# ezwelty/glimpse

Hardware: AMD Instinct MI355X
Metric: particle-frames/s (higher is better)
Workload: dtype f64

## Files before the change

### glimpse_amd/_lib.py

```python
import ctypes as C
import os

import numpy as np

HERE = os.path.dirname(os.path.abspath(__file__))
LIB_PATH = os.environ.get("GLH_LIB") or os.path.join(HERE, "lib", "libglimpse_hip.so")

CAM_LEN = 24
MOTION_LEN = 18
MOTION_FULL_LEN = 24
MOTION_KINDS = {"cartesian": 0, "cylindrical": 1, "tangent_cartesian": 2, "tangent_cylindrical": 3, "external": 4}
RNG_HOST, RNG_PHILOX = 0, 1
MATH_EXACT, MATH_FAST = 0, 1
RESAMPLE = {"systematic": 0, "stratified": 1, "choice": 2, "residual": 3}
OK = 0
PT_NAN, PT_TEMPLATE_OOB, PT_SAMPLE_OUTSIDE, PT_RESAMPLE_CLAMP, PT_CONST_TILE = 1, 2, 4, 8, 16
PT_RASTER_OOB, PT_NOT_VISIBLE = 32, 64
RASTER_DEM, RASTER_DEM_SIGMA, RASTER_VIEWSHED = 0, 1, 2
OBS_OK, OBS_SKIPPED, OBS_OUT_OF_BOUNDS, OBS_TILE_TOO_LARGE, OBS_NO_TEMPLATE = 0, 1, 2, 3, 4
NO_ERROR_FRAME = 0x7F7F7F7F
COMM_ID_BYTES = 128


class GlhError(RuntimeError):
# ... 31 lines not shown
    "glh_sync": (_I, [_P]),
    "glh_get_stream": (_I, [_P, _P]),
    "glh_observer_init": (_I, [_P, _I, _I, _I, _I, _I, _D]),
    "glh_observer_set_cameras": (_I, [_P, _I, _I, _I, _P]),
    "glh_observer_set_depth": (_I, [_P, _I, _I]),
    "glh_observer_upload_frame": (_I, [_P, _I, _I, _P]),
    "glh_observer_upload_frame_async": (_I, [_P, _I, _I, _P]),
    "glh_host_register": (_I, [_P, _U64]),
    "glh_host_unregister": (_I, [_P]),
    "glh_observer_upload_frame_pinned": (_I, [_P, _I, _I, _P, _P]),
    "glh_upload_done": (_I, [_P, C.c_int64, _I, _P]),
    "glh_observer_set_frame_device": (_I, [_P, _I, _I, _P]),
    "glh_begin_sequence": (_I, [_P, _I, _I, _I, _I]),
    "glh_set_motion_cartesian": (_I, [_P, _P]),
    "glh_set_motion": (_I, [_P, _P]),
    "glh_set_raster": (_I, [_P, _I, _P, _I, _I, _P, _P, _I, _I, _D, _D, _D, _D]),
    "glh_set_point_offset": (_I, [_P, _I]),
    "glh_set_observer_mask": (_I, [_P, _P]),
    "glh_set_active": (_I, [_P, _P]),
    "glh_set_particles": (_I, [_P, _P]),
    "glh_get_particles": (_I, [_P, _P]),
    "glh_set_weights": (_I, [_P, _P]),
    "glh_get_weights": (_I, [_P, _P]),
    "glh_set_extra_log_likelihoods": (_I, [_P, _P]),
    "glh_get_point_status": (_I, [_P, _P]),
    "glh_get_point_error_frame": (_I, [_P, _P]),
    "glh_get_observer_status": (_I, [_P, _P]),
    "glh_get_search_boxes": (_I, [_P, _P]),
    "glh_get_observer_status_frames": (_I, [_P, _I, _I, _P]),
    "glh_get_point_state": (_I, [_P, _I, _P, _P]),
    "glh_set_frame": (_I, [_P, _I]),
    "glh_init_particles": (_I, [_P, _I, _P, _U64]),
    "glh_evolve": (_I, [_P, _D, _I, _P, _U64, _U64]),
    "glh_init_templates": (_I, [_P, _I, _I]),
    "glh_update_weights": (_I, [_P, _P]),
    "glh_resample": (_I, [_P, _I, _P, _U64, _U64]),
    "glh_resample_method": (_I, [_P, _I, _I, _P, _U64, _U64]),
    "glh_get_residual_draws": (_I, [_P, _P]),
    "glh_record_covariances": (_I, [_P, _I]),
    "glh_get_covariances": (_I, [_P, _I, _I, _P]),
    "glh_record_moments": (_I, [_P, _I]),
    "glh_step": (_I, [_P, _I, _D, _P, _I, _P, _P, _U64]),
    "glh_track": (_I, [_P, _I, _P, _P, _P, _U64]),
    "glh_track_covariances": (_I, [_P, _I]),
    "glh_set_track_streams": (_I, [_P, _I]),
    "glh_set_fused": (_I, [_P, _I]),
    "glh_set_math": (_I, [_P, _I]),
    "glh_set_highpass": (_I, [_P, _I, _I]),
    "glh_set_highpass_mode": (_I, [_P, _I]),
    "glh_set_interpolation": (_I, [_P, _I, _I]),
    "glh_debug_phase_stamps": (_I, [_P, _P]),
    "glh_debug_draws": (_I, [_P, _I, _U64, _U64, _P]),
    "glh_debug_last_variant": (_I, [_P, _P]),
    "glh_debug_last_track_streams": (_I, [_P, _P]),
    "glh_get_moments": (_I, [_P, _I, _I, _P]),
    "glh_get_tracks": (_I, [_P, _I, _I, _P, _P]),
    "glh_get_moments_device": (_I, [_P, _P, _P]),
    "glh_get_template": (_I, [_P, _I, _I, _P, _P, _P, _P, _P, _P]),
    "glh_get_likelihood_debug": (_I, [_P, _I, _I, _P, _P, _P, _P]),
    "glh_set_debug": (_I, [_P, _I]),
    "glh_get_resample_indices": (_I, [_P, _P]),
    "glh_get_log_likelihoods": (_I, [_P, _I, _P]),
    "glh_profile_enable": (_I, [_P, _I]),
    "glh_profile_reset": (_I, [_P]),
    "glh_stage_count": (_I, []),
    "glh_stage_name": (C.c_char_p, [_I]),
    "glh_profile_get": (_I, [_P, _P, _P]),
    "glh_profile_get_launches": (_I, [_P, _I, _P, _I, _P]),
    "glh_profile_get_span": (_I, [_P, _I, _P]),
    "glh_comm_unique_id": (_I, [_P]),
    "glh_comm_init": (_I, [_P, _P, _I, _I]),
    "glh_comm_destroy": (_I, [_P]),
    "glh_comm_barrier": (_I, [_P]),
    "glh_comm_max_f64": (_I, [_P, _P]),
    "glh_gather_moments": (_I, [_P, _I, _I, _I, _P, _P, _P]),
    "glh_get_gathered": (_I, [_P, _P, _P]),
    "glh_measure_copy_bandwidth": (_I, [_P, _U64, _I, _P]),
    "glh_stage_project": (_I, [_I, _P, _P, _I, _P]),
    "glh_stage_project_directions": (_I, [_I, _P, _P, _I, _P]),
    "glh_stage_project_depth": (_I, [_I, _P, _P, _I, _I, _P, _P]),
    "glh_stage_unproject": (_I, [_I, _P, _P, _I, _P, _I, _I, _P]),
    "glh_stage_reproject": (_I, [_I, _P, _I, _I, _I, _I, _I, _I, _P, _P, _I, _I, _I, _P, _P]),
    "glh_stage_template": (_I, [_I, _P, _I, _I, _I, _P, _P, _P, _P, _P]),
    "glh_stage_search_tile": (_I, [_I, _P, _I, _I, _I, _P, _P, _P, _I, _P]),
    "glh_stage_template_highpass": (_I, [_I, _P, _I, _I, _I, _P, _I, _I, _I, _P, _P, _P, _P]),
    "glh_stage_search_tile_highpass": (_I, [_I, _P, _I, _I, _I, _P, _P, _P, _I, _I, _I, _I, _P]),
    "glh_stage_ssd": (_I, [_I, _P, _I, _I, _P, _I, _I, _P]),
    "glh_stage_sample": (_I, [_I, _P, _I, _I, _P, _P, _I, _P, _P]),
    "glh_stage_sample_orders": (_I, [_I, _P, _I, _I, _I, _I, _P, _P, _I, _P, _P]),
    "glh_stage_resample": (_I, [_I, _P, _I, _D, _P]),
    "glh_stage_raster_sample": (_I, [_I, _P, _I, _I, _P, _P, _I, _I, _D, _D, _D, _D, _P, _I, _I, _P, _P]),
    "glh_stage_viewshed": (_I, [_I, _P, _I, _I, _I, _P, _P, _D, _P, _I, _I, _D, _D, _P, _P]),
    "glh_stage_project_dem": (_I, [_I, _P, _P, _I, _I, _I, _P, _P, _I, _I, _I, _P, _P, _P, _I, _P, _P, _P, _I, _P, _P]),
    "glh_stage_rasterize": (_I, [_I, _P, _I, _P, _I, _I, _P, _P]),
    "glh_stage_max_filter": (_I, [_I, _P, _I, _I, _I, _P, _I, _I, _I, _I, _P, _P]),
    "glh_stage_gaussian_filter": (_I, [_I, _P, _I, _I, _I, _P, _I, _P, _I, _P, _I, _I, _P, _P]),
    "glh_stage_fill_crevasses": (_I, [_I, _P, _I, _I, _I, _P, _I, _I, _I, _I, _P, _I, _P, _I, _I, _P, _P]),
}

_lib = None


def load():
    global _lib
    if _lib is not None:
        return _lib
# ... 293 lines not shown
            uu = _arr(u, np.float64, (self.P,))
            check(self.lib.glh_step(self.handle, int(frame), float(tau), _ptr(im), RNG_HOST, _ptr(n), _ptr(uu), 0))

    def track(self, frames, taus, images, seed=0):
        fr = np.ascontiguousarray(frames, dtype=np.int32).reshape(-1)
        ta = np.ascontiguousarray(taus, dtype=np.float64).reshape(-1)
        im = np.array([[-1 if v is None else int(v) for v in row] for row in images], dtype=np.int32)
        if ta.shape != fr.shape or im.shape != (len(fr), self.O):
            raise ValueError("frames (T,), taus (T,) and images (T, O) do not agree")
        check(self.lib.glh_track(self.handle, len(fr), _ptr(fr), _ptr(ta), _ptr(np.ascontiguousarray(im)), seed))

    def track_covariances(self, on=True):
        check(self.lib.glh_track_covariances(self.handle, int(bool(on))))

    def set_track_streams(self, n):
        check(self.lib.glh_set_track_streams(self.handle, int(n)))

    def last_track_streams(self):
        n = C.c_int(0)
        check(self.lib.glh_debug_last_track_streams(self.handle, C.byref(n)))
        return n.value

    def set_fused(self, mode=1):
        check(self.lib.glh_set_fused(self.handle, int(mode)))

    def set_math(self, mode="exact"):
        check(self.lib.glh_set_math(self.handle, {"exact": MATH_EXACT, "fast": MATH_FAST}[mode]))

    def set_highpass(self, size=(5, 5), mode="reflect"):
        sy, sx = (int(size), int(size)) if np.isscalar(size) else (int(size[0]), int(size[1]))
        check(self.lib.glh_set_highpass(self.handle, sx, sy))
        check(self.lib.glh_set_highpass_mode(self.handle, HIGHPASS_MODES[mode]))

    def set_point_offset(self, offset):
        check(self.lib.glh_set_point_offset(self.handle, int(offset)))

    def phase_stamps(self):
        out = np.zeros((self.P, 24), dtype=np.uint64)
        check(self.lib.glh_debug_phase_stamps(self.handle, _ptr(out)))
        return out

    def debug_draws(self, kind, seed, step=0):
        k = {"init": 0, "evolve": 1, "u": 2}[kind]
        shape = {0: (self.P, self.N, 6), 1: (self.P, self.N, 3), 2: (self.P,)}[k]
        out = np.empty(shape, dtype=np.float64)
        check(self.lib.glh_debug_draws(self.handle, k, int(seed), int(step), _ptr(out)))
        return out

    def last_variant(self):
        out = np.zeros(4, dtype=np.int32)
        check(self.lib.glh_debug_last_variant(self.handle, _ptr(out)))
        return tuple(int(v) for v in out)

    def sync(self):
        check(self.lib.glh_sync(self.handle))

    def stream(self):
        s = C.c_void_p()
        check(self.lib.glh_get_stream(self.handle, C.byref(s)))
        return s.value

    def get_moments(self, frame0, n_frames):
        out = np.empty((n_frames, self.P, 12))
        check(self.lib.glh_get_moments(self.handle, frame0, n_frames, _ptr(out)))
        return out

    def get_tracks(self, frame0, n_frames):
        means, sigmas = np.empty((self.P, n_frames, 6)), np.empty((self.P, n_frames, 6))
        check(self.lib.glh_get_tracks(self.handle, frame0, n_frames, _ptr(means), _ptr(sigmas)))
        return means, sigmas

    def moments_device(self):
        p, n = C.c_void_p(), C.c_uint64()
        check(self.lib.glh_get_moments_device(self.handle, C.byref(p), C.byref(n)))
        return p.value, n.value

    def get_template(self, obs, point):
        tw, th = self.tile
        box = np.empty(4, dtype=np.int32)
        duv = np.empty(2)
        tile = np.empty((th, tw))
        hv = np.empty(tw * th)
        hq = np.empty(tw * th)
        hn = C.c_int32()
        check(self.lib.glh_get_template(self.handle, obs, point, _ptr(box), _ptr(duv), _ptr(tile), _ptr(hv),
                                        _ptr(hq), C.byref(hn)))
        return {"box": box, "duv": duv, "tile": tile, "histogram": (hv[: hn.value].copy(), hq[: hn.value].copy())}

    def set_debug(self, keep=True):
        check(self.lib.glh_set_debug(self.handle, int(keep)))

    def likelihood_debug(self, obs, point, want_sse=True):
        tw, th = self.tile
        uv = np.empty((self.N, 2))
        box = np.empty(4, dtype=np.int32)
        check(self.lib.glh_get_likelihood_debug(self.handle, obs, point, _ptr(uv), _ptr(box), None, None))
        if box[0] < 0:
            return {"uv": uv, "box": None}
        ws, hs = int(box[2] - box[0]), int(box[3] - box[1])
        search = np.empty((hs, ws), dtype=np.float32)
        sse = np.empty((hs - th + 1, ws - tw + 1)) if want_sse else None
        check(self.lib.glh_get_likelihood_debug(self.handle, obs, point, None, None, _ptr(search), _ptr(sse)))
        return {"uv": uv, "box": box, "search": search, "sse": sse}

    def log_likelihoods(self, obs):
        out = np.empty((self.P, self.N))
# ... 370 lines not shown
```

### glimpse_amd/csrc/glh_point.h

```cpp
#pragma once
#include "glh_kernels.h"
#include <type_traits>

namespace glh {

constexpr int PT_MAX_TILE = 63;
constexpr int PT_NSTAMP = GLH_NSTAMP;
constexpr int PT_MAX_OBS = 4;

template <int TB>
__device__ __forceinline__ double pt_block_sum(double v, double* red) {
  v = wave_sum(v);
  __syncthreads();
  if ((threadIdx.x & (WAVE - 1)) == 0) red[threadIdx.x / WAVE] = v;
  __syncthreads();
  double t = red[0];
#pragma unroll
  for (int w = 1; w < TB / WAVE; ++w) t += red[w];
  return t;
}

template <int PPT>
__device__ __forceinline__ double pt_pick(const double (&v)[PPT], int r) {
  double q = v[0];
// ... 54 lines not shown

struct PointArgs {
  const double* particles_in;
  double* particles_out;
  double* weights_tmp;
  double* weights_out;
  const double* motion;
  const uint8_t* obs_mask;
  const double* normals;
  const double* u;
  double* uv;
  int32_t* box;
  int32_t* obs_status;
  const int32_t* tmpl_valid;
  const double* tmpl_duv;
  const float* tmpl_tile32;
  const double* tmpl_hist_v;
  const double* tmpl_hist_q;
  const int32_t* tmpl_hist_n;
  float* ws_search;
  uint16_t* ws_keys;
  double* ws_sse;
  const double* lu;
  const int64_t* lu_off;
  const double* inv;
  const double* poly;
  const uint16_t* uidx_in;
  uint16_t* uidx_out;
  int32_t* idx_out;
  unsigned long long* stamps;
  double* moments;
  uint32_t* pt_status;
  int32_t* pt_err_frame;
  const int32_t* leaf_off;
  const int32_t* leaf_len;
  const int32_t* ops;
  const int32_t* level_off;
  const int32_t* roots;
  uint64_t seed, step;
  double tau;
  double inv2s2[PT_MAX_OBS];
  ObsFrame obs[PT_MAX_OBS];
  CamDev cam[PT_MAX_OBS];
  Surfaces surf;
  uint32_t cam_flags[PT_MAX_OBS];
  int32_t N, P, O, tw, th, tile_cap, search_cap, keys_cap, sse_cap, max_dim, frame, rng_mode, has_dem;
  int32_t hp_rx, hp_ry;
  int32_t interp_k;
  int32_t cell_cap;
  int32_t r2_bytes;
  int32_t pt_base;
  int32_t pt0;
  int32_t stop_at;
  int32_t nleaves, nnodes, nlevels, nroots;
};

__host__ __device__ __forceinline__ int pt_align16(int x) { return (x + 15) & ~15; }
__host__ __device__ __forceinline__ int pt_search_ld(int ws) { return ((ws + 3 + 31) / 32) * 32 + 8; }
__host__ __device__ __forceinline__ int pt_hcl_bytes(int nb) { return pt_align16(nb * 4) + pt_align16(nb * 8); }
__host__ __device__ __forceinline__ int pt_small_bytes(int tw, int th, int nb) {
  return pt_align16(th * ssd_twp(tw) * 4) + pt_hcl_bytes(nb);
}

__host__ __device__ __forceinline__ int pt_keys_stride(int w) { return (w + 6 + 1) & ~1; }
__host__ __device__ __forceinline__ int pt_keys_count(int w, int h) { return (h + 4) * pt_keys_stride(w); }

__host__ __device__ __forceinline__ int pt_park_bytes() { return (13 * 512 + 16) * 8; }

__host__ __device__ __forceinline__ int pt_plan_ints(int nleaves, int nnodes, int nlevels, int nroots) {
  return 2 * nleaves + 3 * (nnodes - nleaves) + (nlevels + 1) + nroots;
}

struct TileWs {
  float* T;
  uint32_t* hist;
  double* lut;
  float* S;
  uint16_t* keys;
  double* Z;
  double* Z1;
  const double* ih;
  const double* iw;
  const double* cdf_q;
  const double* cdf_v;
  const double* fh;
  const double* fw;
  int ld;
};

template <int TB>
__device__ __forceinline__ void pt_border_cols(uint16_t* keys, int wp, int w, int h) {
  for (int idx = threadIdx.x; idx < 5 * h; idx += TB) {
    const int r = idx / 5, k = idx - 5 * r;
    const int c = k < 2 ? -1 - k : w + (k - 2);
    const int src = k < 2 ? k : w - 1 - (k - 2);
    keys[r * wp + c] = keys[r * wp + src];
  }
}
template <int TB>
__device__ __forceinline__ void pt_border_rows(uint16_t* keys, int wp, int h) {
  for (int idx = threadIdx.x; idx < 4 * wp; idx += TB) {
    const int k = idx / wp, c = idx - k * wp - 2;
    const int r = k < 2 ? -1 - k : h + (k - 2);
    const int src = k < 2 ? k : h - 1 - (k - 2);
    keys[r * wp + c] = keys[src * wp + c];
  }
// ... 1121 lines not shown
      } else {
        pt_tile_prep<TB, SURF>(ob, box, nb, hist_n, ws, scan_tmp, (unsigned long long*)a.stamps, a.hp_rx, a.hp_ry);
      }
      PT_STAMP(2);
      if (offT + pt_align16(hs * ws.ld * 4) <= a.r2_bytes) {
        float* Sl = reinterpret_cast<float*>(r2 + offT);
        pt_stage<TB>(reinterpret_cast<float4*>(Sl), reinterpret_cast<const float4*>(ws.S),
                     hs * ws.ld / 4);
        __syncthreads();
        ws.S = Sl;
        pt_ssd<TB>(ws, tw, th, wo, ho);
      } else {
        pt_ssd<TB>(ws, tw, th, wo, ho);
      }
      PT_STAMP(3);
      const int lub = pt_align16(5 * (ho + wo) * 8);
      if (zb + (dense ? zb : lub) <= a.r2_bytes) {
        double* Zl = reinterpret_cast<double*>(r2);
        double* fl = Zl + zb / 8;
        pt_stage<TB>(Zl, static_cast<const double*>(ws.Z), ho * wo);
        if (need_lu) {
          for (int k = tid; k < 5 * ho; k += TB) fl[k] = fh_g[k];
          for (int k = tid; k < 5 * wo; k += TB) fl[5 * ho + k] = fw_g[k];
          ws.fh = fl;
          ws.fw = fl + 5 * ho;
        }
        __syncthreads();
        ws.Z = Zl;
        ws.Z1 = fl;
        if (!linear) pt_spline_fit<TB>(ws, wo, ho);
        PT_STAMP(4);
        if (!to_cells(Zl)) sample_all(Zl, std::false_type{});
      } else {
        if (dense) ws.Z1 = reinterpret_cast<double*>(r2);
        if (!linear) pt_spline_fit<TB>(ws, wo, ho);
        PT_STAMP(4);
        sample_all(ws.Z, std::false_type{});
      }
    }
    if (cells) sample_all(reinterpret_cast<const double*>(r2), std::true_type{});
    __syncthreads();
  }
  if (!c_ready) {
    if (SURF && !motion_term) {
      for (int i = tid; i < N; i += TB) c[i] = W[uin ? (int)uin[i] : i];
      w_done = true;
      __syncthreads();
    } else {
      for (int i = tid; i < N; i += TB) c[i] = 0.0;
    }
  }
  PT_STAMP(5);
  if (outside) flag_point(a.pt_status, a.pt_err_frame, pt, GLH_PT_SAMPLE_OUTSIDE, a.frame);
  if (!w_done) {
    const bool mterm = a.has_dem && motion_term;
    double wn = mterm ? W[tid < N ? tid : 0] : 0.0;
    for (int i = tid; i < N; i += TB) {
      double ll = c[i];
      const double wi = wn;
      if (mterm) wn = W[i + TB < N ? i + TB : 0];
      if (mterm) ll += wi;
      c[i] = weight_of<FAST>(ll, tab32);
    }
    __syncthreads();
  }

  PT_STAMP(6);
  double* node = reinterpret_cast<double*>(r2);
  double total = 1.0;
  if constexpr (!FAST) {
    {
      const int sub = tid & 7;
      for (int L = tid >> 3; L < a.nleaves; L += TB / 8) {
        const int off = p_leaf_off[L], len = p_leaf_len[L];
        double res;
        if (len < 8) {
          res = 0.0;
          if (sub == 0)
            for (int i = 0; i < len; ++i) res += c[off + i];
        } else {
          double r = c[off + sub];
          const int body = len - (len & 7);
          for (int i = 8; i < body; i += 8) r += c[off + i + sub];
          r += __shfl_xor(r, 1, WAVE);
          r += __shfl_xor(r, 2, WAVE);
          r += __shfl_xor(r, 4, WAVE);
          res = r;
          if (sub == 0)
            for (int i = body; i < len; ++i) res += c[off + i];
        }
        if (sub == 0) node[L] = res;
      }
    }
    __syncthreads();
    for (int l = 0; l < a.nlevels; ++l) {
      for (int k = p_level_off[l] + tid; k < p_level_off[l + 1]; k += TB) {
        const int32_t* op = p_ops + 3 * k;
        node[op[0]] = node[op[1]] + node[op[2]];
      }
      __syncthreads();
    }
    total = node[p_roots[0]];
    for (int r = 1; r < a.nroots; ++r) total += node[p_roots[r]];
  }
  PT_STAMP(10);
  const int seg = (N + TB - 1) / TB;
  const int k0 = min(tid * seg, N), k1 = min(k0 + seg, N);
  double run = 0.0;
  double qn[NREG];
  if constexpr (PPT > 0 && FAST && (NREG & 1) == 0) {
    if (seg == NREG && N % seg == 0) {
      const double2* c2 = reinterpret_cast<const double2*>(c + (k0 < N ? k0 : 0));
#pragma unroll
      for (int j = 0; j < NREG; j += 2) {
        const double2 q = c2[j >> 1];
        qn[j] = k0 < N ? q.x : 0.0;
        qn[j + 1] = k0 < N ? q.y : 0.0;
        run += qn[j];
        run += qn[j + 1];
      }
    } else {
#pragma unroll
      for (int j = 0; j < NREG; ++j) {
        qn[j] = k0 + j < k1 ? c[k0 + j] : 0.0;
        if (k0 + j < k1) run += qn[j];
      }
    }
  } else if constexpr (PPT > 0) {
#pragma unroll
    for (int j = 0; j < NREG; ++j) {
      qn[j] = k0 + j < k1 ? (FAST ? c[k0 + j] : c[k0 + j] / total) : 0.0;
      if (k0 + j < k1) run += qn[j];
    }
  } else {
    for (int k = k0; k < k1; ++k) run += FAST ? c[k] : c[k] / total;
  }
  double incl = run, prev;
  if constexpr (FAST) {
    incl = wave_scan_add_f64(run);
    prev = wave_shr1_f64(incl);
  } else {
#pragma unroll
    for (int off = 1; off < WAVE; off <<= 1) {
      double t = __shfl_up(incl, off, WAVE);
      if (lane >= off) incl += t;
    }
    prev = __shfl_up(incl, 1, WAVE);
    if (lane == 0) prev = 0.0;
  }
  if (lane == WAVE - 1) wave_tot[wave] = incl;
  __syncthreads();
  double base = 0.0;
  for (int w = 0; w < wave; ++w) base += wave_tot[w];
  const double excl = base + prev;
  PT_STAMP(11);
  const int n16 = pt_align16(N * 2) / 2;
  uint16_t* ufill = reinterpret_cast<uint16_t*>(r2);
  uint32_t* usc = reinterpret_cast<uint32_t*>(ufill + n16);
  const int tables_bytes = pt_align16(n16 * 2 + N * 4);
  const bool clast_behind = tables_bytes + TB * (int)sizeof(double) <= a.r2_bytes;
  double* clast = clast_behind ? reinterpret_cast<double*>(r2 + tables_bytes) : node + a.nnodes;
  clast[tid] = tid > 0 ? excl + run : run;
  if (FAST && tid == TB - 1) s_scale = (double)N / (excl + run);
  if (clast_behind)
    for (int q = tid; q < n16 / 8; q += TB) reinterpret_cast<uint4*>(ufill)[q] = make_uint4(0u, 0u, 0u, 0u);
  PT_STAMP(12);
  const double u = s_u;
  const double inv_n = 1.0 / (double)N;
  __shared__ int s_U;
  {
    const double dN = (double)N;
    pt_lds_barrier();
    const double pos_scale = FAST ? s_scale : 0.0;
    auto count_le = [&](double ck) -> int {
      if constexpr (FAST) return count_le_fast(ck, pos_scale, u, N);
      double g = floor(ck * dN - u) + 1.0;
      g = g < 0.0 ? 0.0 : (g > dN ? dN : g);
      const bool below_ok = !(g > 0.0) || ((g - 1.0) + u) * inv_n <= ck;
      const bool above_ok = !(g < dN) || !((g + u) * inv_n <= ck);
      int f = (int)g;
      if (!(below_ok && above_ok)) {
        while (f < N && ((double)f + u) * inv_n <= ck) ++f;
        while (f > 0 && ((double)(f - 1) + u) * inv_n > ck) --f;
      }
      return f;
    };
    const int f_first = k0 > 0 && k0 < N ? count_le(clast[tid - 1]) : 0;
    int fk[NREG];
    int nsurv = 0;
    {
      int f_prev = f_first;
      double run2 = 0.0;
      if constexpr (PPT > 0) {
#pragma unroll
        for (int j = 0; j < NREG; ++j) {
          const int k = k0 + j;
          fk[j] = f_prev;
          if (k < k1) {
            run2 += qn[j];
            int f = count_le(tid > 0 ? excl + run2 : run2);
            if (k == N - 1 && f < N) {
              flag_point(a.pt_status, a.pt_err_frame, pt, GLH_PT_RESAMPLE_CLAMP, a.frame);
              f = N;
            }
            nsurv += f > f_prev;
            f_prev = f;
            fk[j] = f;
          }
        }
      } else {
        for (int k = k0; k < k1; ++k) {
          run2 += FAST ? c[k] : c[k] / total;
          int f = count_le(tid > 0 ? excl + run2 : run2);
          if (k == N - 1 && f < N) {
            flag_point(a.pt_status, a.pt_err_frame, pt, GLH_PT_RESAMPLE_CLAMP, a.frame);
            f = N;
          }
          nsurv += f > f_prev;
          f_prev = f;
        }
      }
    }
    const int incl_s = (int)wave_scan_add_u32((uint32_t)nsurv);
    if (lane == WAVE - 1) scan_tmp[wave] = (uint32_t)incl_s;
    pt_lds_barrier();
    int rank = incl_s - nsurv;
    for (int w = 0; w < wave; ++w) rank += (int)scan_tmp[w];
    if (tid == TB - 1) s_U = rank + nsurv;
    if (!clast_behind) {
      for (int q = tid; q < n16 / 8; q += TB) reinterpret_cast<uint4*>(ufill)[q] = make_uint4(0u, 0u, 0u, 0u);
      pt_lds_barrier();
    }
    {
      int f_prev = f_first;
      double run2 = 0.0;
      if constexpr (PPT > 0) {
#pragma unroll
        for (int j = 0; j < NREG; ++j) {
          const int k = k0 + j;
          if (k < k1) {
            const int f = fk[j];
            if (f > f_prev) {
              usc[rank] = (uint32_t)k | ((uint32_t)(f - f_prev) << 16);
              ufill[f_prev] = (uint16_t)(rank + 1);
              ++rank;
            }
            f_prev = f;
          }
        }
      } else {
        for (int k = k0; k < k1; ++k) {
          run2 += FAST ? c[k] : c[k] / total;
          int f = count_le(tid > 0 ? excl + run2 : run2);
          if (k == N - 1 && f < N) f = N;
          if (f > f_prev) {
            usc[rank] = (uint32_t)k | ((uint32_t)(f - f_prev) << 16);
            ufill[f_prev] = (uint16_t)(rank + 1);
            ++rank;
          }
          f_prev = f;
        }
      }
    }
    pt_lds_barrier();
    if (s_U == 0 && tid == 0) {
      usc[0] = (uint32_t)N << 16;
      ufill[0] = 1;
    }
    constexpr int MS_W = 5;
    const bool words = (seg & 1) == 0 && seg <= 2 * MS_W && N % seg == 0;
    uint32_t* segw = reinterpret_cast<uint32_t*>(ufill + k0);
    uint32_t wv[MS_W];
    uint32_t runmax = 0;
    if (words) {
#pragma unroll
      for (int q = 0; q < MS_W; ++q) {
        wv[q] = 0;
        if (2 * q < seg && k0 < N) {
          const uint32_t w = segw[q];
          const uint32_t lo = max(w & 0xffffu, runmax), hi = max(w >> 16, lo);
          runmax = hi;
          wv[q] = lo | (hi << 16);
        }
      }
    } else {
      for (int j = k0; j < k1; ++j) {
        runmax = max(runmax, (uint32_t)ufill[j]);
        ufill[j] = (uint16_t)runmax;
      }
    }
    const uint32_t incl_m = wave_scan_max_u32(runmax);
    if (lane == WAVE - 1) scan_tmp[wave] = incl_m;
    uint32_t before = wave_shr1_u32(incl_m);
    pt_lds_barrier();
    for (int w = 0; w < wave; ++w) before = max(before, scan_tmp[w]);
    if (words) {
      const glh_us2 bb = {(unsigned short)before, (unsigned short)before};
#pragma unroll
      for (int q = 0; q < MS_W; ++q)
        if (2 * q < seg && k0 < N)
          segw[q] = __builtin_bit_cast(uint32_t, __builtin_elementwise_max(__builtin_bit_cast(glh_us2, wv[q]), bb));
    } else if (before > 0) {
      for (int j = k0; j < k1; ++j) ufill[j] = (uint16_t)max((uint32_t)ufill[j], before);
    }
  }
  pt_lds_barrier();

  PT_STAMP(7);
  double* Pout = a.particles_out + (size_t)pt * N * 6;
  double* Wout = a.weights_out + (size_t)pt * N;
  const int U = max(s_U, 1);
  double K[6];
#pragma unroll
  for (int k = 0; k < 6; ++k) K[k] = s_K[k];
  double s0 = 0.0, s1[6] = {0, 0, 0, 0, 0, 0}, s2[6] = {0, 0, 0, 0, 0, 0};
  constexpr int GU = SURF ? 1 : (TB >= 1024 ? 3 : 2);
  uint32_t sc_n[GU];
  int rec_n[GU];
  double zp_n[GU];
  auto fetch_next = [&](int h0) {
#pragma unroll
    for (int g = 0; g < GU; ++g) {
      const int h = h0 + g * TB;
      sc_n[g] = h < U ? usc[h] : 0u;
      rec_n[g] = COMMON || uin ? (int)uin[sc_n[g] & 0xffffu] : (int)(sc_n[g] & 0xffffu);
      zp_n[g] = GRID && tangent_pt ? ZP[sc_n[g] & 0xffffu] : 0.0;
    }
  };
  fetch_next(tid);
  for (int h0 = tid; h0 < U; h0 += GU * TB) {
    int lo[GU], cnt[GU];
    double2 v[GU][3];
    double zp[GU];
#pragma unroll
    for (int g = 0; g < GU; ++g) {
      lo[g] = (int)(sc_n[g] & 0xffffu);
      cnt[g] = (int)(sc_n[g] >> 16);
      const double2* src = Pin2 + (size_t)rec_n[g] * rec_stride;
      v[g][0] = src[0]; v[g][1] = src[chunk_stride]; v[g][2] = src[2 * chunk_stride];
      zp[g] = zp_n[g];
    }
    fetch_next(h0 + GU * TB);
#pragma unroll
    for (int g = 0; g < GU; ++g) {
      if (g) asm volatile("" ::: "memory");
      double x[6] = {v[g][0].x, v[g][0].y, v[g][1].x, v[g][1].y, v[g][2].x, v[g][2].y};
      evolve_loaded(lo[g], x, zp[g]);
      const double w = c[lo[g]];
      const int h = h0 + g * TB;
      if (h < U) {
        typedef double pt_d2 __attribute__((ext_vector_type(2)));
        pt_d2* dst = reinterpret_cast<pt_d2*>(Pout) + h;
        __builtin_nontemporal_store(pt_d2{x[0], x[1]}, dst);
        __builtin_nontemporal_store(pt_d2{x[2], x[3]}, dst + N);
        __builtin_nontemporal_store(pt_d2{x[4], x[5]}, dst + 2 * N);
        __builtin_nontemporal_store(w, Wout + h);
        const double cw = (double)cnt[g] * w;
        s0 += cw;
#pragma unroll
        for (int k = 0; k < 6; ++k) {
          double d = x[k] - K[k];
          double wd = cw * d;
          if constexpr (FAST) {
            s1[k] = glh_fma(cw, d, s1[k]);
            s2[k] = glh_fma(wd, d, s2[k]);
          } else {
            s1[k] += wd;
            s2[k] += wd * d;
          }
        }
      }
    }
  }
  {
    uint16_t* uout = a.uidx_out + (size_t)pt * N;
    if (!a.idx_out && (N & 7) == 0) {
      const glh_us2 one = {1, 1};
      for (int q = tid; q < N / 8; q += TB) {
        uint4 v = reinterpret_cast<const uint4*>(ufill)[q];
        uint32_t* w = reinterpret_cast<uint32_t*>(&v);
#pragma unroll
        for (int k = 0; k < 4; ++k)
          w[k] = __builtin_bit_cast(uint32_t, __builtin_elementwise_max(__builtin_bit_cast(glh_us2, w[k]), one) - one);
        reinterpret_cast<uint4*>(uout)[q] = v;
      }
    } else {
      for (int j = tid; j < N; j += TB) {
        const int h = max((int)ufill[j], 1) - 1;
        uout[j] = (uint16_t)h;
        if (a.idx_out) a.idx_out[(size_t)pt * N + j] = (int32_t)(usc[h] & 0xffffu);
      }
    }
  }
  PT_STAMP(8);
  {
    pt_lds_barrier();
    constexpr int NP = 512;
    double* M = c;
    if constexpr (TB > NP) {
      static_assert(TB == 2 * NP, "lane pairs");
      s0 = group_sum_dpp(s0, 2);
#pragma unroll
      for (int k = 0; k < 6; ++k) {
        s1[k] = group_sum_dpp(s1[k], 2);
        s2[k] = group_sum_dpp(s2[k], 2);
      }
    }
    if (TB == NP || !(tid & 1)) {
      const int slot = TB == NP ? tid : tid >> 1;
// ... 40 lines not shown
```

### glimpse_amd/csrc/glimpse_hip.hip

```cpp
#include <hip/hip_runtime.h>

#include <algorithm>
#include <cmath>
#include <cstdarg>
#include <cstdio>
#include <cstdlib>
#include <cstring>
#include <string>
#include <vector>

#include "../../include/glimpse_hip.h"
#include "glh_comm.h"
#include "glh_host.h"
#include "glh_kernels.h"
#include "glh_point.h"
#include "glh_point_variants.h"
#include "glh_project_dem.h"
#include "glh_viewshed.h"
#include "glh_filters.h"

using namespace glh;

namespace glh {
#define GLH_PT_DECL(TB, PPT, NOBS, S, F, C) const void* GLH_PT_NAME(TB, PPT, NOBS, S, F, C)();
// ... 1399 lines not shown
  c->moments_frame = c->have_active ? -1 : c->frame;
  return GLH_OK;
}

extern "C" int glh_record_moments(glh_ctx* c, int frame) {
  CHK(need_seq(c));
  HIPCHK(hipSetDevice(c->cfg.device_id));
  if (frame < 0 || frame >= c->cfg.max_frames) return fail(GLH_E_INVALID, "frame %d outside [0, max_frames)", frame);
  if (c->moments_frame == frame && !c->have_active) return GLH_OK;
  return launch_moments(c, c->moments + (size_t)frame * c->P * 12, 12, 1);
}


static bool fused_plan(const glh_ctx* c, int* r2_bytes, int mode = -1) {
  if (mode < 0) mode = c->fused;
  const int O = c->cfg.n_observers;
  if (O > PT_MAX_OBS || c->tw > PT_MAX_TILE || c->th > PT_MAX_TILE) return false;
  if (c->interp_k == 0) return false;

  int nb = 256;
  for (int o = 0; o < O; ++o) {
    if (c->obs[o].channels != 1 && c->obs[o].channels != 3) return false;
    if (c->obs[o].bits >= 16 && c->cfg.max_search_dim > 255) return false;
    if (c->obs[o].channels == 3 || c->obs[o].bits >= 16) nb = 766;
  }
  const int cN = pt_align16(c->N * 8) + pt_align16(4 * pt_plan_ints(c->nleaves, c->nnodes, c->nlevels, c->nroots));
  const int plan = std::max(pt_align16(c->nnodes * 8) + PT_BLK_BIG * 8, 3 * pt_align16(c->N * 2));
  const int r2_min = std::max(plan, std::max(pt_small_bytes(c->tw, c->th, nb) + GLH_SPL_DENSE_NINV / 2 * 8,
                                             pt_align16(GLH_SPL_DENSE_MAX * GLH_SPL_DENSE_MAX * 8)));
  const int typical = pt_small_bytes(c->tw, c->th, nb) + 48 * pt_search_ld(48) * 4 + pt_keys_count(48, 48) * 2;
  const int patch = c->rasters[0].z || c->rasters[1].z || c->rasters[2].z ? PT_PATCH_LDS : 0;
  const int lds_half = PT_LDS_HALF - patch, lds_max = PT_LDS_MAX - patch;
  int r2;
  if (cN + std::max(r2_min, typical) <= lds_half)
    r2 = lds_half - cN;
  else
    r2 = std::min(lds_max - cN, 72 * 1024);
  if (mode == 2) r2 = r2_min;
  if (r2 < r2_min || cN + r2 > lds_max) return false;
  *r2_bytes = r2;
  return true;
}

static int cell_cap(const glh_ctx* c) {
  int r2 = 0;
  if (!fused_plan(c, &r2, c->fused == 2 ? 2 : 1)) return 0;
  int tb, ppt;
  pt_shape(c->N, c->cfg.n_observers, &tb, &ppt);
  return std::min(r2 / (GLH_CELL_LD * 8), 2 * tb / 4);
}

static int fused_step(glh_ctx* c, int frame, double tau, const int32_t* images, int rng_mode, const double* u,
                      uint64_t seed, int r2_bytes, int pt0 = 0, int npts = -1, hipStream_t on = nullptr,
                      bool flip = true) {
  const int O = c->cfg.n_observers;
  if (npts < 0) npts = c->P;
  if (!on) on = c->stream;
  if (rng_mode == GLH_RNG_HOST) {
    if (!u) return fail(GLH_E_INVALID, "GLH_RNG_HOST needs u [P]");
    HIPCHK(hipMemcpyAsync(c->u, u, (size_t)c->P * sizeof(double), hipMemcpyHostToDevice, c->stream));
    HIPCHK(hipStreamSynchronize(c->stream));
  }
  PointArgs a{};
  a.particles_in = c->particles[c->cur];
  a.particles_out = c->particles[c->cur ^ 1];
  a.weights_tmp = c->weights[c->cur];
  a.weights_out = c->weights[c->cur ^ 1];
  a.motion = c->motion;
  a.obs_mask = c->have_mask ? c->obs_mask : nullptr;
  a.normals = c->normals;
  a.u = c->u;
  a.uv = c->uv;
  a.box = c->box;
  a.obs_status = cur_status(c);
  a.tmpl_valid = c->tmpl_valid;
  a.tmpl_duv = c->tmpl_duv;
  a.tmpl_tile32 = c->tmpl_tile32;
  a.tmpl_hist_v = c->tmpl_hist_v;
  a.tmpl_hist_q = c->tmpl_hist_q;
  a.tmpl_hist_n = c->tmpl_hist_n;
  a.ws_search = c->search;
  a.ws_keys = c->ws_keys;
  a.ws_sse = c->sse;
  a.lu = c->lu;
  a.lu_off = c->lu_off;
  a.inv = c->spl_inv;
  a.poly = c->poly;
  a.idx_out = c->keep_idx ? c->idx : nullptr;
  for (int b = 0; b < 2; ++b)
    if (!c->uidx[b]) CHK(dalloc(&c->uidx[b], (size_t)c->cfg.max_points * c->cfg.max_particles));
  a.uidx_in = c->compact ? c->uidx[c->cur] : nullptr;
  a.uidx_out = c->uidx[c->cur ^ 1];
  a.stamps = c->stamps ? c->stamps + (size_t)pt0 * PT_NSTAMP : nullptr;
  a.pt0 = pt0;
  a.moments = c->moments + (size_t)frame * c->P * 12;
  a.pt_status = c->pt_status;
  a.pt_err_frame = c->pt_err_frame;
  a.leaf_off = c->leaf_off;
  a.leaf_len = c->leaf_len;
  a.ops = c->sum_ops;
  a.level_off = c->level_off;
  a.roots = c->roots;
  a.seed = seed;
  a.step = (uint64_t)frame;
  a.tau = tau;
  for (int o = 0; o < O; ++o) {
    if (c->obs[o].bits >= 32) CHK(prepare_bins16(c, o, true));
    fill_obs(c, o, images[o], &a.obs[o]);
    if ((int)c->obs[o].cams_host.size() != c->obs[o].n_images)
      return fail(GLH_E_STATE, "observer %d: cameras have not been set", o);
    a.cam[o] = c->obs[o].cams_host[images[o] >= 0 ? images[o] : 0];
    a.cam_flags[o] = cam_flags(a.cam[o]);
    a.inv2s2[o] = 1.0 / (2.0 * (c->obs[o].sigma * c->obs[o].sigma));
  }
  a.N = c->N;
  a.P = c->P;
  a.O = O;
  a.tw = c->tw;
  a.th = c->th;
  a.tile_cap = c->tile_cap;
  a.search_cap = c->search_cap;
  a.keys_cap = c->keys_cap;
  a.sse_cap = c->sse_cap;
  a.max_dim = c->cfg.max_search_dim;
  a.frame = frame;
  a.rng_mode = rng_mode;
  a.has_dem = c->has_dem;
  a.r2_bytes = r2_bytes;
  a.cell_cap = cell_cap(c);
  a.hp_rx = c->hp_rx;
  a.hp_ry = c->hp_ry;
  a.interp_k = c->interp_k;
  a.pt_base = c->pt_base;
  a.stop_at = c->stop_frame == frame ? c->stop_stamp : -1;
  a.surf = surfaces(c);
  a.nleaves = c->nleaves;
  a.nnodes = c->nnodes;
  a.nlevels = c->nlevels;
  a.nroots = c->nroots;
  {
    StageTimer t(c, ST_POINT_STEP, on);
    const size_t lds = std::max((size_t)pt_align16(c->N * 8) + r2_bytes +
                                    pt_align16(4 * pt_plan_ints(c->nleaves, c->nnodes, c->nlevels, c->nroots)),
                                (size_t)pt_park_bytes());
    const dim3 grid(npts);
    int tb, ppt;
    pt_shape(c->N, O, &tb, &ppt);
    const dim3 block(tb);
    const bool fast = use_fast(c);
    bool common = fast && rng_mode == GLH_RNG_PHILOX && c->compact && !c->have_mask;
    for (int o = 0; o < O; ++o) common &= a.obs[o].on && !(a.cam_flags[o] & CAM_F_NOT_SIMPLE);
    bool plain = c->hp_rx == 2 && c->hp_ry == 2 && c->interp_k == 3;
    for (int o = 0; o < O; ++o) plain &= c->obs[o].bits == 8;
    const bool rast = c->rasters[0].z || c->rasters[1].z || c->rasters[2].z;
    const bool surf = rast || !c->all_cartesian || (fast && !common) || !plain;
    c->last_variant[0] = tb; c->last_variant[1] = ppt; c->last_variant[2] = O;
    c->last_variant[3] = (fast ? 1 : 0) | (surf ? 2 : 0) | (common ? 4 : 0) | (rast ? 8 : 0);
    const void* kern = pt_kernel(tb, ppt, O, rast ? 2 : (surf ? 1 : 0), fast, surf ? common : fast);
    if (!kern) return fail(GLH_E_STATE, "no instantiation of the fused kernel for <%d, %d, %d>", tb, ppt, O);
    void* kargs[] = {(void*)&a};
    HIPCHK(hipLaunchKernel(kern, grid, block, kargs, lds, on));
  }
  HIPCHK(hipGetLastError());
  if (flip) {
    c->cur ^= 1;
    c->compact = true;
    c->moments_frame = frame;
  }
  return GLH_OK;
}

extern "C" int glh_get_residual_draws(glh_ctx* c, int32_t* draws) {
  CHK(need_seq(c));
  if (!draws) return fail(GLH_E_INVALID, "null argument");
  if (!c->resid_draws) return fail(GLH_E_STATE, "no residual resampling has run");
  DOWNLOAD(draws, c->resid_draws, (size_t)c->P, int32_t);
  return GLH_OK;
}

extern "C" int glh_record_covariances(glh_ctx* c, int frame) {
  CHK(need_seq(c));
  HIPCHK(hipSetDevice(c->cfg.device_id));
  if (frame < 0 || frame >= c->cfg.max_frames) return fail(GLH_E_INVALID, "frame %d outside [0, max_frames)", frame);
  if (!c->covariances) {
    const size_t n = (size_t)c->cfg.max_frames * c->cfg.max_points * 36;
    CHK(dalloc(&c->covariances, n));
    hipLaunchKernelGGL(k_fill_f64, dim3(256), dim3(256), 0, c->stream, c->covariances, n, (double)NAN);
// ... 40 lines not shown
    return fused_step(c, frame, tau, images, rng_mode, u, seed, r2_bytes);
  CHK(launch_evolve_project(c, true, tau, rng_mode, seed, (uint64_t)frame, images));
  CHK(update_weights_impl(c, images, true));
  CHK(glh_resample(c, rng_mode, u, seed, (uint64_t)frame));
  return glh_record_moments(c, frame);
}

extern "C" int glh_track(glh_ctx* c, int n_frames, const int32_t* frames, const double* taus, const int32_t* images,
                         uint64_t seed) {
  CHK(need_seq(c));
  if (n_frames <= 0 || !frames || !taus || !images)
    return fail(GLH_E_INVALID, "n_frames must be > 0 and the arrays non-null");
  const int O = c->cfg.n_observers;
  for (int k = 0; k < n_frames; ++k) {
    if (frames[k] < 0 || frames[k] >= c->cfg.max_frames)
      return fail(GLH_E_INVALID, "frame %d outside [0, max_frames)", frames[k]);
    CHK(check_images(c, images + (size_t)k * O));
  }
  int r2_bytes = 0;
  const bool fused_ok = c->fused && !c->have_active && !c->keep_sse && !c->have_extra && fused_plan(c, &r2_bytes);
  int ns = 1;
  if (fused_ok && !c->track_covariances) {
    if (c->track_streams >= 2) ns = c->track_streams;
    else if (c->track_streams == 0 && c->P > c->n_cus) ns = 2;
    ns = std::min(ns, c->P);
  }
  c->last_track_streams = ns;
  if (ns == 1) {
    int rc = GLH_OK;
    for (int k = 0; k < n_frames && rc == GLH_OK; ++k) {
      rc = glh_step(c, frames[k], taus[k], images + (size_t)k * O, GLH_RNG_PHILOX, nullptr, nullptr, seed);
      if (rc == GLH_OK && c->track_covariances) rc = glh_record_covariances(c, frames[k]);
    }
    return rc;
  }
  HIPCHK(hipSetDevice(c->cfg.device_id));
  if (!c->ev_fork) HIPCHK(hipEventCreateWithFlags(&c->ev_fork, hipEventDisableTiming));
  hipStream_t on[4] = {c->stream, nullptr, nullptr, nullptr};
  for (int q = 1; q < ns; ++q) {
    if (!c->extra_streams[q - 1]) {
      HIPCHK(hipStreamCreateWithFlags(&c->extra_streams[q - 1], hipStreamNonBlocking));
      HIPCHK(hipEventCreateWithFlags(&c->ev_join[q - 1], hipEventDisableTiming));
    }
    on[q] = c->extra_streams[q - 1];
  }
  HIPCHK(hipEventRecord(c->ev_fork, c->stream));
  for (int q = 1; q < ns; ++q) HIPCHK(hipStreamWaitEvent(on[q], c->ev_fork, 0));
  int rc = GLH_OK;
  for (int k = 0; k < n_frames && rc == GLH_OK; ++k) {
    rc = glh_set_frame(c, frames[k]);
    for (int q = 0; q < ns && rc == GLH_OK; ++q) {
      const int p0 = (int)((int64_t)c->P * q / ns), p1 = (int)((int64_t)c->P * (q + 1) / ns);
      rc = fused_step(c, frames[k], taus[k], images + (size_t)k * O, GLH_RNG_PHILOX, nullptr, seed, r2_bytes, p0,
                      p1 - p0, on[q], q == ns - 1);
    }
  }
  for (int q = 1; q < ns; ++q) {
    (void)hipEventRecord(c->ev_join[q - 1], on[q]);
    (void)hipStreamWaitEvent(c->stream, c->ev_join[q - 1], 0);
  }
  return rc;
}

extern "C" int glh_set_track_streams(glh_ctx* c, int n) {
  if (!c) return fail(GLH_E_INVALID, "null context");
  if (n < 0 || n > 4) return fail(GLH_E_INVALID, "streams must be 0 (automatic) or 1 .. 4");
  c->track_streams = n;
  return GLH_OK;
}

extern "C" int glh_debug_last_track_streams(glh_ctx* c, int* n) {
  if (!c || !n) return fail(GLH_E_INVALID, "null argument");
  *n = c->last_track_streams;
  return GLH_OK;
}

extern "C" int glh_track_covariances(glh_ctx* c, int on) {
  if (!c) return fail(GLH_E_INVALID, "null context");
  c->track_covariances = on != 0;
  return GLH_OK;
}

extern "C" int glh_measure_copy_bandwidth(glh_ctx* c, uint64_t bytes, int iters, double* gbps) {
  if (!c || !gbps || bytes == 0 || iters <= 0) return fail(GLH_E_INVALID, "bad argument");
  HIPCHK(hipSetDevice(c->cfg.device_id));
  uint8_t *src = nullptr, *dst = nullptr;
  CHK(dalloc(&src, (size_t)bytes));
  if (dalloc(&dst, (size_t)bytes) != GLH_OK) {
    dfree(src);
    return GLH_E_NOMEM;
  }
  hipEvent_t e0 = nullptr, e1 = nullptr;
  float ms = 0.0f;
  hipError_t err = hipMemsetAsync(src, 1, bytes, c->stream);
  if (err == hipSuccess) err = hipMemcpyAsync(dst, src, bytes, hipMemcpyDeviceToDevice, c->stream);
  if (err == hipSuccess) err = hipEventCreate(&e0);
  if (err == hipSuccess) err = hipEventCreate(&e1);
  if (err == hipSuccess) err = hipEventRecord(e0, c->stream);
  for (int k = 0; k < iters && err == hipSuccess; ++k)
    err = hipMemcpyAsync(dst, src, bytes, hipMemcpyDeviceToDevice, c->stream);
  if (err == hipSuccess) err = hipEventRecord(e1, c->stream);
  if (err == hipSuccess) err = hipEventSynchronize(e1);
  if (err == hipSuccess) err = hipEventElapsedTime(&ms, e0, e1);
  if (e0) (void)hipEventDestroy(e0);
  if (e1) (void)hipEventDestroy(e1);
  dfree(src);
  dfree(dst);
  if (err != hipSuccess) return fail(GLH_E_HIP, "copy bandwidth measurement failed: %s", hipGetErrorString(err));
  *gbps = 2.0 * (double)bytes * iters / ((double)ms * 1e-3) / 1e9;
  return GLH_OK;
}

extern "C" int glh_debug_last_variant(glh_ctx* c, int32_t* variant) {
  if (!c || !variant) return fail(GLH_E_INVALID, "null argument");
  for (int k = 0; k < 4; ++k) variant[k] = c->last_variant[k];
  return GLH_OK;
}

extern "C" int glh_debug_draws(glh_ctx* c, int kind, uint64_t seed, uint64_t step, double* out) {
  CHK(need_seq(c));
  if (!out || kind < 0 || kind > 2) return fail(GLH_E_INVALID, "kind must be 0 (init), 1 (evolve) or 2 (resample offset)");
  HIPCHK(hipSetDevice(c->cfg.device_id));
  const size_t per = kind == 0 ? 6 : (kind == 1 ? 3 : 0);
  const size_t count = kind == 2 ? (size_t)c->P : (size_t)c->P * c->N * per;
  double* buf = nullptr;
  CHK(dalloc(&buf, count));
  DrawsArgs a{};
  a.out = buf;
  a.seed = seed;
  a.step = step;
  a.kind = kind;
  a.N = c->N;
  a.P = c->P;
  a.pt_base = c->pt_base;
  hipLaunchKernelGGL(k_debug_draws, dim3(kind == 2 ? 1 : (c->N + BLK - 1) / BLK, c->P), dim3(BLK), 0, c->stream, a);
  hipError_t e = hipGetLastError();
  if (e == hipSuccess) e = hipMemcpyAsync(out, buf, count * sizeof(double), hipMemcpyDeviceToHost, c->stream);
  if (e == hipSuccess) e = hipStreamSynchronize(c->stream);
  dfree(buf);
  if (e != hipSuccess) return fail(GLH_E_HIP, "glh_debug_draws failed: %s", hipGetErrorString(e));
  return GLH_OK;
}

extern "C" int glh_debug_phase_stamps(glh_ctx* c, uint64_t* stamps) {
  CHK(need_seq(c));
  if (!stamps) return fail(GLH_E_INVALID, "null argument");
  HIPCHK(hipSetDevice(c->cfg.device_id));
  const size_t n = (size_t)c->P * PT_NSTAMP;
  if (!c->stamps) {
    CHK(dalloc(&c->stamps, (size_t)c->cfg.max_points * PT_NSTAMP));
    HIPCHK(hipMemset(c->stamps, 0, (size_t)c->cfg.max_points * PT_NSTAMP * sizeof(unsigned long long)));
    memset(stamps, 0, n * sizeof(uint64_t));
    return GLH_OK;
  }
  DOWNLOAD(stamps, c->stamps, n, unsigned long long);
  return GLH_OK;
}

extern "C" int glh_set_highpass(glh_ctx* c, int size_x, int size_y) {
  if (!c) return fail(GLH_E_INVALID, "null context");
  if (size_x < 1 || size_y < 1 || size_x > 7 || size_y > 7 || !(size_x & 1) || !(size_y & 1))
    return fail(GLH_E_UNSUPPORTED, "high-pass window %d x %d: sizes must be odd and at most 7", size_x, size_y);
// ... 1058 lines not shown
```

### include/glimpse_hip.h

```cpp
#ifndef GLIMPSE_HIP_H
#define GLIMPSE_HIP_H

#include <stdint.h>

#ifdef __cplusplus
extern "C" {
#endif

#define GLH_VERSION 100

#define GLH_OK 0
#define GLH_E_INVALID (-1)
#define GLH_E_HIP (-2)
#define GLH_E_NOMEM (-3)
#define GLH_E_STATE (-4)
#define GLH_E_UNSUPPORTED (-5)
#define GLH_E_COMM (-6)

#define GLH_CAM_LEN 24

#define GLH_MOTION_LEN 18

#define GLH_MOTION_FULL_LEN 24
#define GLH_MOTION_CARTESIAN 0
// ... 66 lines not shown
int glh_begin_sequence(glh_ctx* ctx, int n_points, int n_particles, int tile_w, int tile_h);
int glh_set_motion_cartesian(glh_ctx* ctx, const double* params);
int glh_set_motion(glh_ctx* ctx, const double* params);
#define GLH_RASTER_DEM 0
#define GLH_RASTER_DEM_SIGMA 1
#define GLH_RASTER_VIEWSHED 2
int glh_set_raster(glh_ctx* ctx, int which, const double* z, int nx, int ny, const double* gx,
                   const double* gy, int sx, int sy, double xmin, double xmax, double ymin, double ymax);
int glh_set_point_offset(glh_ctx* ctx, int offset);
int glh_set_observer_mask(glh_ctx* ctx, const uint8_t* mask);
int glh_set_active(glh_ctx* ctx, const uint8_t* active);

int glh_set_particles(glh_ctx* ctx, const double* particles);
int glh_get_particles(glh_ctx* ctx, double* particles);
int glh_set_weights(glh_ctx* ctx, const double* weights);
int glh_set_extra_log_likelihoods(glh_ctx* ctx, const double* ll);
int glh_get_weights(glh_ctx* ctx, double* weights);
int glh_get_point_status(glh_ctx* ctx, uint32_t* status);
int glh_get_point_error_frame(glh_ctx* ctx, int32_t* frames);
int glh_get_observer_status(glh_ctx* ctx, int32_t* status);
int glh_get_observer_status_frames(glh_ctx* ctx, int frame0, int n_frames, int32_t* status);
int glh_get_point_state(glh_ctx* ctx, int point, double* particles, double* weights);
int glh_get_search_boxes(glh_ctx* ctx, int32_t* boxes);

int glh_set_frame(glh_ctx* ctx, int frame);
int glh_init_particles(glh_ctx* ctx, int rng_mode, const double* normals, uint64_t seed);
int glh_evolve(glh_ctx* ctx, double tau, int rng_mode, const double* normals, uint64_t seed,
               uint64_t step);
int glh_init_templates(glh_ctx* ctx, int obs, int image);
int glh_update_weights(glh_ctx* ctx, const int32_t* images );
int glh_resample(glh_ctx* ctx, int rng_mode, const double* u, uint64_t seed, uint64_t step);
int glh_resample_method(glh_ctx* ctx, int method, int rng_mode, const double* u, uint64_t seed,
                        uint64_t step);
int glh_get_residual_draws(glh_ctx* ctx, int32_t* draws);
int glh_record_covariances(glh_ctx* ctx, int frame);
int glh_get_covariances(glh_ctx* ctx, int frame0, int n_frames, double* out);
int glh_record_moments(glh_ctx* ctx, int frame);
int glh_step(glh_ctx* ctx, int frame, double tau, const int32_t* images, int rng_mode,
             const double* normals, const double* u, uint64_t seed);
int glh_track(glh_ctx* ctx, int n_frames, const int32_t* frames, const double* taus, const int32_t* images,
              uint64_t seed);
int glh_track_covariances(glh_ctx* ctx, int on);
int glh_set_track_streams(glh_ctx* ctx, int n);

int glh_set_fused(glh_ctx* ctx, int on);
int glh_set_math(glh_ctx* ctx, int mode);
int glh_set_highpass(glh_ctx* ctx, int size_x, int size_y);
int glh_set_highpass_mode(glh_ctx* ctx, int mode);
int glh_set_interpolation(glh_ctx* ctx, int kx, int ky);

int glh_debug_draws(glh_ctx* ctx, int kind, uint64_t seed, uint64_t step, double* out);
int glh_debug_phase_stamps(glh_ctx* ctx, uint64_t* stamps);
int glh_debug_last_variant(glh_ctx* ctx, int32_t* variant);
int glh_debug_last_track_streams(glh_ctx* ctx, int* n);

int glh_get_moments(glh_ctx* ctx, int frame0, int n_frames, double* out);
int glh_get_tracks(glh_ctx* ctx, int frame0, int n_frames, double* means, double* sigmas);
int glh_get_moments_device(glh_ctx* ctx, void** dev_ptr, uint64_t* bytes);
int glh_get_template(glh_ctx* ctx, int obs, int point, int32_t* box, double* duv, double* tile,
                     double* hist_values, double* hist_quantiles, int32_t* hist_n);
int glh_get_likelihood_debug(glh_ctx* ctx, int obs, int point, double* uv, int32_t* box,
                             float* search, double* sse);
int glh_set_debug(glh_ctx* ctx, int keep);
int glh_get_log_likelihoods(glh_ctx* ctx, int obs, double* ll);
int glh_get_resample_indices(glh_ctx* ctx, int32_t* idx);
int glh_profile_enable(glh_ctx* ctx, int on);
int glh_profile_reset(glh_ctx* ctx);
int glh_stage_count(void);
const char* glh_stage_name(int stage);
int glh_profile_get(glh_ctx* ctx, double* ms , int64_t* launches );
int glh_profile_get_span(glh_ctx* ctx, int stage, double* ms);
int glh_profile_get_launches(glh_ctx* ctx, int stage, double* ms, int cap, int* n);
int glh_measure_copy_bandwidth(glh_ctx* ctx, uint64_t bytes, int iters, double* gbps);

#define GLH_COMM_ID_BYTES 128
int glh_comm_unique_id(char* id );
int glh_comm_init(glh_ctx* ctx, const char* id, int rank, int world);
int glh_comm_destroy(glh_ctx* ctx);
int glh_comm_barrier(glh_ctx* ctx);
int glh_comm_max_f64(glh_ctx* ctx, double* value);
int glh_gather_moments(glh_ctx* ctx, int root, int frame0, int n_frames, const int32_t* points_per_rank,
                       double* out, uint32_t* status);
int glh_get_gathered(glh_ctx* ctx, double* out, uint32_t* status);

int glh_stage_project(int device_id, const double* cam, const double* xyz, int n, double* uv);
int glh_stage_project_directions(int device_id, const double* cam, const double* xyz, int n, double* uv);
int glh_stage_project_depth(int device_id, const double* cam, const double* xyz, int n, int directions,
                            double* uv, double* depth);
int glh_stage_unproject(int device_id, const double* cam, const double* uv, int n, const double* depth,
                        int n_depth, int directions, double* xyz);
int glh_stage_reproject(int device_id, const void* frames, int depth_bits, int is_float, int width, int height,
                        int channels, int n_frames, const double* src_cams, const double* dst_cam, int dst_width,
                        int dst_height, int method, void* out, double* kernel_ms);
int glh_stage_template(int device_id, const uint8_t* frame, int width, int height, int channels,
                       const int32_t* box, double* tile, double* hist_values,
                       double* hist_quantiles, int32_t* hist_n);
int glh_stage_search_tile(int device_id, const uint8_t* frame, int width, int height,
                          int channels, const int32_t* box, const double* hist_values,
                          const double* hist_quantiles, int hist_n, float* tile);
int glh_stage_template_highpass(int device_id, const uint8_t* frame, int width, int height, int channels,
                                const int32_t* box, int size_x, int size_y, int mode, double* tile,
                                double* hist_values, double* hist_quantiles, int32_t* hist_n);
int glh_stage_search_tile_highpass(int device_id, const uint8_t* frame, int width, int height, int channels,
                                   const int32_t* box, const double* hist_values, const double* hist_quantiles,
                                   int hist_n, int size_x, int size_y, int mode, float* tile);
int glh_stage_ssd(int device_id, const float* search, int hs, int ws, const float* templ, int th,
// ... 41 lines not shown
```

Before: 45.93 billion.

## Cache resample record indices in LDS and skip intermediate weight stores in track

During the fused resample, each unique draw's record index is now computed when the draw table is built and stored in a spare region of shared scratch. The output loop then reads it from there instead of doing a dependent gather through uin. Threads whose segment is evenly aligned preload their uin values as packed 32-bit words. Separately, glh_track now writes particle weights to global memory only on the last frame (or when surfaces are on), which cuts nontemporal store traffic on intermediate frames. The trade-offs are extra LDS use and register pressure, plus a reliance on intermediate weights never being read between frames. A debug API to fetch record indices is also added.

Result: no change. 46.00 billion, median of 5 (+0.1%).

```diff
diff --git a/glimpse_amd/_lib.py b/glimpse_amd/_lib.py
--- a/glimpse_amd/_lib.py
+++ b/glimpse_amd/_lib.py
@@ -107,6 +107,7 @@
     "glh_debug_phase_stamps": (_I, [_P, _P]),
     "glh_debug_draws": (_I, [_P, _I, _U64, _U64, _P]),
     "glh_debug_last_variant": (_I, [_P, _P]),
+    "glh_debug_record_indices": (_I, [_P, _P]),
     "glh_debug_last_track_streams": (_I, [_P, _P]),
     "glh_get_moments": (_I, [_P, _I, _I, _P]),
     "glh_get_tracks": (_I, [_P, _I, _I, _P, _P]),
@@ -506,6 +507,11 @@
         check(self.lib.glh_debug_last_variant(self.handle, _ptr(out)))
         return tuple(int(v) for v in out)
 
+    def record_indices(self):
+        out = np.zeros((self.P, self.N), dtype=np.uint16)
+        check(self.lib.glh_debug_record_indices(self.handle, _ptr(out)))
+        return out
+
     def sync(self):
         check(self.lib.glh_sync(self.handle))
 
diff --git a/glimpse_amd/csrc/glh_point.h b/glimpse_amd/csrc/glh_point.h
--- a/glimpse_amd/csrc/glh_point.h
+++ b/glimpse_amd/csrc/glh_point.h
@@ -130,6 +130,7 @@
   int32_t pt_base;
   int32_t pt0;
   int32_t stop_at;
+  int32_t store_weights;
   int32_t nleaves, nnodes, nlevels, nroots;
 };
 
@@ -1357,6 +1358,17 @@
   }
   PT_STAMP(5);
   if (outside) flag_point(a.pt_status, a.pt_err_frame, pt, GLH_PT_SAMPLE_OUTSIDE, a.frame);
+  const int seg = (N + TB - 1) / TB;
+  const int k0 = min(tid * seg, N), k1 = min(k0 + seg, N);
+  constexpr int RECW = PPT > 0 ? (NREG + 1) / 2 : 1;
+  uint32_t recw[RECW] = {};
+  const bool rec_words = PPT > 0 && (COMMON || uin) && (seg & 1) == 0 && N % seg == 0;
+  if (rec_words) {
+    const uint32_t* uw32 = reinterpret_cast<const uint32_t*>(uin + (k0 < N ? k0 : 0));
+#pragma unroll
+    for (int q = 0; q < RECW; ++q) recw[q] = 2 * q < seg ? uw32[q] : 0u;
+  }
+  auto rec_of = [&](int k) -> uint16_t { return COMMON || uin ? uin[k] : (uint16_t)k; };
   if (!w_done) {
     const bool mterm = a.has_dem && motion_term;
     double wn = mterm ? W[tid < N ? tid : 0] : 0.0;
@@ -1409,8 +1421,6 @@
     for (int r = 1; r < a.nroots; ++r) total += node[p_roots[r]];
   }
   PT_STAMP(10);
-  const int seg = (N + TB - 1) / TB;
-  const int k0 = min(tid * seg, N), k1 = min(k0 + seg, N);
   double run = 0.0;
   double qn[NREG];
   if constexpr (PPT > 0 && FAST && (NREG & 1) == 0) {
@@ -1462,7 +1472,10 @@
   const int n16 = pt_align16(N * 2) / 2;
   uint16_t* ufill = reinterpret_cast<uint16_t*>(r2);
   uint32_t* usc = reinterpret_cast<uint32_t*>(ufill + n16);
-  const int tables_bytes = pt_align16(n16 * 2 + N * 4);
+  const int usc_end = pt_align16(n16 * 2 + N * 4);
+  const int urec_cap = min(max(a.r2_bytes - usc_end, 0) / 2, N);
+  uint16_t* urec = reinterpret_cast<uint16_t*>(r2 + usc_end);
+  const int tables_bytes = usc_end;
   const bool clast_behind = tables_bytes + TB * (int)sizeof(double) <= a.r2_bytes;
   double* clast = clast_behind ? reinterpret_cast<double*>(r2 + tables_bytes) : node + a.nnodes;
   clast[tid] = tid > 0 ? excl + run : run;
@@ -1547,6 +1560,7 @@
             const int f = fk[j];
             if (f > f_prev) {
               usc[rank] = (uint32_t)k | ((uint32_t)(f - f_prev) << 16);
+              if (rank < urec_cap) urec[rank] = rec_words ? (uint16_t)(recw[j >> 1] >> (16 * (j & 1))) : rec_of(k);
               ufill[f_prev] = (uint16_t)(rank + 1);
               ++rank;
             }
@@ -1560,6 +1574,7 @@
           if (k == N - 1 && f < N) f = N;
           if (f > f_prev) {
             usc[rank] = (uint32_t)k | ((uint32_t)(f - f_prev) << 16);
+            if (rank < urec_cap) urec[rank] = rec_of(k);
             ufill[f_prev] = (uint16_t)(rank + 1);
             ++rank;
           }
@@ -1570,6 +1585,7 @@
     pt_lds_barrier();
     if (s_U == 0 && tid == 0) {
       usc[0] = (uint32_t)N << 16;
+      if (urec_cap > 0) urec[0] = rec_of(0);
       ufill[0] = 1;
     }
     constexpr int MS_W = 5;
@@ -1614,6 +1630,7 @@
   PT_STAMP(7);
   double* Pout = a.particles_out + (size_t)pt * N * 6;
   double* Wout = a.weights_out + (size_t)pt * N;
+  const bool store_w = SURF || a.store_weights != 0;
   const int U = max(s_U, 1);
   double K[6];
 #pragma unroll
@@ -1628,7 +1645,7 @@
     for (int g = 0; g < GU; ++g) {
       const int h = h0 + g * TB;
       sc_n[g] = h < U ? usc[h] : 0u;
-      rec_n[g] = COMMON || uin ? (int)uin[sc_n[g] & 0xffffu] : (int)(sc_n[g] & 0xffffu);
+      rec_n[g] = h < urec_cap ? (h < U ? (int)urec[h] : 0) : (int)rec_of((int)(sc_n[g] & 0xffffu));
       zp_n[g] = GRID && tangent_pt ? ZP[sc_n[g] & 0xffffu] : 0.0;
     }
   };
@@ -1659,7 +1676,7 @@
         __builtin_nontemporal_store(pt_d2{x[0], x[1]}, dst);
         __builtin_nontemporal_store(pt_d2{x[2], x[3]}, dst + N);
         __builtin_nontemporal_store(pt_d2{x[4], x[5]}, dst + 2 * N);
-        __builtin_nontemporal_store(w, Wout + h);
+        if (store_w) __builtin_nontemporal_store(w, Wout + h);
         const double cw = (double)cnt[g] * w;
         s0 += cw;
 #pragma unroll
diff --git a/glimpse_amd/csrc/glimpse_hip.hip b/glimpse_amd/csrc/glimpse_hip.hip
--- a/glimpse_amd/csrc/glimpse_hip.hip
+++ b/glimpse_amd/csrc/glimpse_hip.hip
@@ -1475,7 +1475,7 @@
 
 static int fused_step(glh_ctx* c, int frame, double tau, const int32_t* images, int rng_mode, const double* u,
                       uint64_t seed, int r2_bytes, int pt0 = 0, int npts = -1, hipStream_t on = nullptr,
-                      bool flip = true) {
+                      bool flip = true, bool store_weights = true) {
   const int O = c->cfg.n_observers;
   if (npts < 0) npts = c->P;
   if (!on) on = c->stream;
@@ -1556,6 +1556,7 @@
   a.interp_k = c->interp_k;
   a.pt_base = c->pt_base;
   a.stop_at = c->stop_frame == frame ? c->stop_stamp : -1;
+  a.store_weights = store_weights;
   a.surf = surfaces(c);
   a.nleaves = c->nleaves;
   a.nnodes = c->nnodes;
@@ -1702,7 +1703,7 @@
     for (int q = 0; q < ns && rc == GLH_OK; ++q) {
       const int p0 = (int)((int64_t)c->P * q / ns), p1 = (int)((int64_t)c->P * (q + 1) / ns);
       rc = fused_step(c, frames[k], taus[k], images + (size_t)k * O, GLH_RNG_PHILOX, nullptr, seed, r2_bytes, p0,
-                      p1 - p0, on[q], q == ns - 1);
+                      p1 - p0, on[q], q == ns - 1, k == n_frames - 1);
     }
   }
   for (int q = 1; q < ns; ++q) {
@@ -1758,6 +1759,20 @@
   dfree(dst);
   if (err != hipSuccess) return fail(GLH_E_HIP, "copy bandwidth measurement failed: %s", hipGetErrorString(err));
   *gbps = 2.0 * (double)bytes * iters / ((double)ms * 1e-3) / 1e9;
+  return GLH_OK;
+}
+
+extern "C" int glh_debug_record_indices(glh_ctx* c, uint16_t* out) {
+  CHK(need_seq(c));
+  if (!out) return fail(GLH_E_INVALID, "null argument");
+  if (c->compact) {
+    DOWNLOAD(out, c->uidx[c->cur], (size_t)c->P * c->N, uint16_t);
+  } else {
+    HIPCHK(hipSetDevice(c->cfg.device_id));
+    HIPCHK(hipStreamSynchronize(c->stream));
+    for (int p = 0; p < c->P; ++p)
+      for (int i = 0; i < c->N; ++i) out[(size_t)p * c->N + i] = (uint16_t)i;
+  }
   return GLH_OK;
 }
 
diff --git a/include/glimpse_hip.h b/include/glimpse_hip.h
--- a/include/glimpse_hip.h
+++ b/include/glimpse_hip.h
@@ -142,6 +142,7 @@
 int glh_debug_draws(glh_ctx* ctx, int kind, uint64_t seed, uint64_t step, double* out);
 int glh_debug_phase_stamps(glh_ctx* ctx, uint64_t* stamps);
 int glh_debug_last_variant(glh_ctx* ctx, int32_t* variant);
+int glh_debug_record_indices(glh_ctx* ctx, uint16_t* out);
 int glh_debug_last_track_streams(glh_ctx* ctx, int* n);
 
 int glh_get_moments(glh_ctx* ctx, int frame0, int n_frames, double* out);
```
